# alexandervakhitov/lld-slam

Measured on AMD Instinct MI355X. Metric: local-BA windows/sec (50 KF, 10k pts, 2k lines) at matched chi2; 1/2/4/8 GPU, higher is better.
Workload: dtype f64; 1 GPU; batched LocalBundleAdjustment, 256 LBA-B windows per GPU (50 free + 10 fixed KF, 10k points x 6 stereo obs, 2k lines x 5 KF x 2 images = 80k edges), 5+15 LM iterations, gamma=1; windows resident in HBM, every step restarts from the uploaded state; bit_reproducible=True, windows_per_gpu=256, edges_per_window=80000, parallelism=1 x independent window batches, RCCL gather of result records, resident=True

## Files before the change

lld_slam_amd/csrc/lld_ba_control.h:

```cpp

__device__ __forceinline__ void ba_control_body(const BAArrays& A, const BAWin& W, BAState& S, int lane, int n_windows, int abort_flag,
                                                int wrow , int nw_group ,
                                                int* __restrict__ counters ,
                                                int* __restrict__ host_counters ,
                                                const int* __restrict__ host_abort ) {
  double tempChi = 0.0, scale_l = 0.0;
  int do_clear = 0;
  const bool valid = wrow >= 0;
  if (valid) {
  if (S.phase == PH_RUN) {
    const int nb = W.nt_pt + W.nt_ln;
    for (int i = lane; i < nb; i += 64) { tempChi += xwg_load(&A.chi_part2[W.part_off + i]); scale_l += xwg_load(&A.scale_part[W.part_off + i]); }
    tempChi = lld_wave::sum(tempChi); scale_l = lld_wave::sum(scale_l);
  }
  if (lane == 0 && S.phase == PH_RUN) {
    double scale = S.scale_cam + scale_l;
    if (!S.pcg_ok) tempChi = 1.7976931348623157e308;
    double rho = (S.currentChi - tempChi);
    scale += 1e-3;
    rho /= scale;
    if (rho > 0 && isfinite(tempChi)) {
      double alpha = 1. - (2 * rho - 1) * (2 * rho - 1) * (2 * rho - 1);
      alpha = fmin(alpha, 2. / 3.);
      S.lambda *= fmax(1. / 3., alpha);
      S.ni = 2;
      S.currentChi = tempChi;
      S.cur ^= 1;
    } else {
      S.lambda *= S.ni; S.ni *= 2;
    }
    S.q++;
    const int round = S.round;
    S.lm_trials[round]++;
    const bool stop = abort_flag || (host_abort && __hip_atomic_load(host_abort, __ATOMIC_RELAXED, __HIP_MEMORY_SCOPE_SYSTEM) != 0) ||
                      (W.abort_after > 0 && S.lm_trials[0] + S.lm_trials[1] >= W.abort_after);
    const bool again = (rho < 0 && S.q < W.max_trials && !stop);
    if (!again) {
      bool term = (S.q == W.max_trials || rho == 0);
      if (!term) {
        if ((S.iniChi - S.currentChi) * 1e3 < S.iniChi) S.nBad++; else S.nBad = 0;
        if (S.nBad >= 3) term = true;
      }
      S.it++;
      S.lm_iterations[round]++;
      if (!term && S.it < W.its[round] && !stop) { S.need_lin = 1; S.maxdiag_bits = 0ull; do_clear = 1; }
      else if (round == 0) {
        S.chi2_round1 = S.currentChi; S.chi2_final = S.currentChi;
        if (stop) { S.aborted = 1; S.phase = PH_FINALIZE; }
        else if (W.protocol == 1) S.phase = PH_FINALIZE;
        else S.phase = PH_TRANSITION;
      } else { S.chi2_final = S.currentChi; S.aborted = stop ? 1 : 0; S.phase = PH_FINALIZE; }
    }
  }
  do_clear = __builtin_amdgcn_readfirstlane(do_clear);
  if (do_clear) {
    for (int i = lane; i < W.n_free * 21; i += 64) A.Hpp[(size_t)W.hpp_off * 21 + i] = 0.0;
    for (int i = lane; i < W.n_free * 6; i += 64) A.bp[(size_t)W.hpp_off * 6 + i] = 0.0;
    if (W.big) for (int i = lane; i < W.n_free * 27; i += 64) A.hpp_part[W.hpart_off + i] = 0.0;
  }
  }
  int last = 0;
  if (lane == 0) {
    if (valid) {
      const int ph = S.phase;
      if (ph == PH_RUN) atomicAdd(&counters[0], 1);
      else if (ph == PH_TRANSITION) atomicAdd(&counters[1], 1);
      else if (ph == PH_FINALIZE) atomicAdd(&counters[2], 1);
      if (A.slot_map) { xwg_store_i32(&A.active_pub[wrow], (ph == PH_RUN || ph == PH_TRANSITION) ? 1 : 0); xwg_stores_done(); }
    }
    if (atomicAdd(&counters[3], 1) == n_windows - 1) {
#pragma unroll
      for (int i = 0; i < 3; i++) {
        const int v = atomicExch(&counters[i], 0);
// ... 4 lines not shown
      last = 1;
    }
  }
  last = __builtin_amdgcn_readfirstlane(last);
  if (last && A.slot_map) {
    int cnt = 0;
    for (int base = 0; base < nw_group; base += 64) {
      const int w = base + lane;
      const bool act = w < nw_group && xwg_load_i32(&A.active_pub[w]) != 0;
      const unsigned long long m = __ballot(act);
      if (act) A.slot_map[cnt + __popcll(m & ((1ull << lane) - 1ull))] = w;
      cnt += __popcll(m);
    }
    for (int k = cnt + lane; k < nw_group; k += 64) A.slot_map[k] = -1;
  }
}
__global__ __launch_bounds__(kCtlThreads) void ba_control_kernel(BAArrays A, const BAWin* __restrict__ wins, BAState* __restrict__ st, int abort_flag, int nw_group,
                                                                 int* __restrict__ counters, int* __restrict__ host_counters, const int* __restrict__ host_abort) {
  const int wrow = LLD_ROW_WINDOW(A, st, blockIdx.x);
  const int wi = wrow < 0 ? 0 : wrow;
  ba_control_body(A, wins[wi], st[wi], threadIdx.x, (int)gridDim.x, abort_flag, wrow, nw_group, counters, host_counters, host_abort);
}

__global__ __launch_bounds__(kLmThreads) void ba_backsub_ctl_kernel(BAArrays A, const BAWin* __restrict__ wins, BAState* __restrict__ st, int n_pt_blocks, int abort_flag, int nw_group,
                                                                   int* __restrict__ counters, int* __restrict__ host_counters, const int* __restrict__ host_abort) {
  __shared__ int is_last;
  const int wrow = LLD_ROW_WINDOW(A, st, blockIdx.y);
  const int bx = (int)blockIdx.x;
  if (wrow < 0) {
    if (bx == 0 && threadIdx.x < 64) ba_control_body(A, wins[0], st[0], threadIdx.x, (int)gridDim.y, abort_flag, -1, nw_group, counters, host_counters, host_abort);
    return;
  }
  const BAWin& W = wins[wrow];
  BAState& S = st[wrow];
  const bool running = S.phase == PH_RUN;
  const bool is_pt = bx < n_pt_blocks;
  const bool works = running && (is_pt ? bx < W.nt_pt : bx - n_pt_blocks < W.nt_ln);
  if (works) {
    if (is_pt) ba_backsub_pt_body<false, 1>(A, wins, st, bx); else ba_backsub_ln_body<false, 1>(A, wins, st, bx - n_pt_blocks);
  }
  if (!running) {
    if (bx == 0 && threadIdx.x < 64) ba_control_body(A, W, S, threadIdx.x, (int)gridDim.y, abort_flag, wrow, nw_group, counters, host_counters, host_abort);
    return;
  }
  if (!works) return;
  if (threadIdx.x == 0) is_last = atomicAdd(&S.ticket_bs, 1) == W.nt_pt + W.nt_ln - 1;
  __syncthreads();
  if (is_last && threadIdx.x < 64) {
    if (threadIdx.x == 0) S.ticket_bs = 0;
    ba_control_body(A, W, S, threadIdx.x, (int)gridDim.y, abort_flag, wrow, nw_group, counters, host_counters, host_abort);
  }
}

__global__ __launch_bounds__(kLmThreads) void ba_classify_kernel(BAArrays A, const BAWin* __restrict__ wins, BAState* __restrict__ st) {
  __shared__ double scratch[8];
  const int wrow = LLD_ROW_WINDOW(A, st, blockIdx.y);
  if (wrow < 0) return;
  const BAWin W = wins[wrow];
  BAState& S = st[wrow];
  if (S.phase != PH_TRANSITION) return;
  if ((int)blockIdx.x >= W.nb_pt + W.nb_ln) return;
  const int cur = S.cur;
  const CamK cam = W.cam;
  double n_active = 0.0;
  if ((int)blockIdx.x < W.nb_pt) {
    const int p0 = blockIdx.x * kLmThreads, np = min(kLmThreads, W.n_pt - p0);
    const int eb = A.pt_obs_start[W.pt_off + p0], ee = A.pt_obs_start[W.pt_off + p0 + np];
    for (int e = eb + (int)threadIdx.x; e < ee; e += kLmThreads) {
      uint8_t fl = A.pe_flags[e];
      const Vec3 X = load_pt(A, cur, W.pt_off + A.pe_pt[e]);
      const Pose T = load_cam(A, cur, W.cam_off + pt_cam_of<kPkRuntime>(A, e));
      const bool depth_pos = pose_map(T, X).z > 0.0;
      const bool stereo = pt_obs_stereo<kPkRuntime>(A, e);
      if (A.pe_chi2[e] > (stereo ? 7.815 : 5.991) || !depth_pos) fl |= EF_LEVEL1;
      fl &= (uint8_t)~EF_ROBUST;
      A.pe_flags[e] = fl;
    }
    __syncthreads();
    const int p = p0 + threadIdx.x;
    if (p < W.n_pt) {
      const int g = W.pt_off + p;
      int act = 0;
      for (int e = A.pt_obs_start[g]; e < A.pt_obs_start[g + 1]; e++) act += !(A.pe_flags[e] & EF_LEVEL1);
      A.pt_active[g] = act > 0;
      n_active += act;
    }
  } else {
    const int l0 = (blockIdx.x - W.nb_pt) * kLmThreads, nl = min(kLmThreads, W.n_ln - l0);
    const int eb = 2 * A.ln_obs_start[W.ln_off + l0], ee = 2 * A.ln_obs_start[W.ln_off + l0 + nl];
    for (int e = eb + (int)threadIdx.x; e < ee; e += kLmThreads) {
      uint8_t fl = A.le_flags[e];
      if (!(fl & EF_VALID)) continue;
      const LineQ L = load_ln(A, cur, W.ln_off + ln_line_of<kPkRuntime>(A, e >> 1));
      const Mat3 Rl = line_rotation(L);
      const Vec3 c0 = mat_col(Rl, 0), c1 = mat_col(Rl, 1);
      const double th = (fl & EF_PAIRSTEREO) ? W.th_ln_stereo : W.th_ln_mono;
      const Pose T = load_cam(A, cur, W.cam_off + ln_cam_of<kPkRuntime>(A, e >> 1));
      const LnSeg sg = ln_seg_of<kPkRuntime>(A, e);
      const bool depth_pos = line_depth_positive(cam, (e & 1) ? cam.bx_right : 0.0, T, c0, c1, L.alpha, sg.xs, sg.ys, sg.xe, sg.ye);
      if (A.le_chi2[e] > th * th || !depth_pos) fl |= EF_LEVEL1;
      fl &= (uint8_t)~EF_ROBUST;
      A.le_flags[e] = fl;
    }
    __syncthreads();
    const int l = l0 + threadIdx.x;
    if (l < W.n_ln) {
      const int g = W.ln_off + l;
      const int e0 = 2 * A.ln_obs_start[g], e1 = 2 * A.ln_obs_start[g + 1];
      int cnt = 0, act = 0; bool has_edge = false;
      for (int e = e0; e < e1; e++) {
        const uint8_t fl = A.le_flags[e];
        if (!(fl & EF_VALID)) continue;
        has_edge = true;
        if (!(fl & EF_LEVEL1)) { cnt += 2; act++; }
      }
      const bool removed = has_edge && cnt <= W.ln_filter;
      if (removed) {
        for (int e = e0; e < e1; e++) if (A.le_flags[e] & EF_VALID) A.le_flags[e] |= EF_LEVEL1;
        act = 0;
      }
      A.ln_removed[g] = removed;
      A.ln_active[g] = act > 0;
      n_active += act;
    }
  }
  const double t = block_sum(n_active, scratch);
  __shared__ int is_last;
  if (threadIdx.x == 0) {
    if (t > 0.0) atomicAdd(&S.n_active_edges, (int)(t + 0.5));
    is_last = atomicAdd(&S.ticket_cls, 1) == W.nb_pt + W.nb_ln - 1;
  }
  __syncthreads();
  if (!is_last) return;
  for (int i = threadIdx.x; i < W.n_free * 21; i += kLmThreads) A.Hpp[(size_t)W.hpp_off * 21 + i] = 0.0;
  for (int i = threadIdx.x; i < W.n_free * 6; i += kLmThreads) A.bp[(size_t)W.hpp_off * 6 + i] = 0.0;
  if (W.big) for (int i = threadIdx.x; i < W.n_free * 27; i += kLmThreads) A.hpp_part[W.hpart_off + i] = 0.0;
  __syncthreads();
  if (threadIdx.x == 0) {
    S.ticket_cls = 0;
    S.round = 1; S.it = 0; S.q = 0; S.need_lin = 1; S.maxdiag_bits = 0ull;
    S.phase = __hip_atomic_load(&S.n_active_edges, __ATOMIC_RELAXED, __HIP_MEMORY_SCOPE_AGENT) > 0 ? PH_RUN : PH_FINALIZE;
  }
}

struct BARecordHeader {
  double chi2_round1, chi2_final;
  int lm_iterations[2], lm_trials[2];
  int pcg_iterations, aborted, win_index, n_pt_obs;
};
__device__ __forceinline__ double* rec_cam(unsigned char* r) { return reinterpret_cast<double*>(r + sizeof(BARecordHeader)); }

__global__ __launch_bounds__(kLmThreads) void ba_finalize_kernel(BAArrays A, const BAWin* __restrict__ wins, const BAState* __restrict__ st) {
  const BAWin W = wins[blockIdx.y];
  const BAState& S = st[blockIdx.y];
  if (S.phase != PH_FINALIZE) return;
  if ((int)blockIdx.x >= W.nb_pt + W.nb_ln + 1) return;
  const int cur = S.cur;
  const CamK cam = W.cam;
  const bool global = W.protocol == 1;
  const bool untouched = S.aborted && S.lm_trials[0] == 0;
  unsigned char* rec = A.records + W.rec_off;
  double* o_cam = rec_cam(rec);
  double* o_pt = o_cam + 7 * W.n_cams;
  double* o_x0 = o_pt + 3 * W.n_pt;
  double* o_dir = o_x0 + 3 * W.n_ln;
  unsigned char* o_pe = reinterpret_cast<unsigned char*>(o_dir + 3 * W.n_ln);
  unsigned char* o_le = o_pe + W.n_pe;
  unsigned char* o_rm = o_le + W.n_le;
  if ((int)blockIdx.x == W.nb_pt + W.nb_ln) {
    for (int i = threadIdx.x; i < W.n_cams * 7; i += kLmThreads) o_cam[i] = A.cam_qt[((size_t)cur * A.NC + W.cam_off) * 7 + i];
    if (threadIdx.x == 0) {
      BARecordHeader h;
      h.chi2_round1 = S.chi2_round1; h.chi2_final = S.chi2_final;
      h.lm_iterations[0] = S.lm_iterations[0]; h.lm_iterations[1] = S.lm_iterations[1];
      h.lm_trials[0] = S.lm_trials[0]; h.lm_trials[1] = S.lm_trials[1];
      h.pcg_iterations = S.pcg_iterations; h.aborted = S.aborted; h.win_index = W.win_index; h.n_pt_obs = W.n_pe;
      *reinterpret_cast<BARecordHeader*>(rec) = h;
    }
    return;
  }
  if ((int)blockIdx.x < W.nb_pt) {
    const int p = blockIdx.x * kLmThreads + threadIdx.x;
    if (p < W.n_pt) {
      const Vec3 X = load_pt(A, cur, W.pt_off + p);
      o_pt[3 * p] = X.x; o_pt[3 * p + 1] = X.y; o_pt[3 * p + 2] = X.z;
    }
    for (int e = W.pe_off + p; e < W.pe_off + W.n_pe; e += W.nb_pt * kLmThreads) {
      const Vec3 X = load_pt(A, cur, W.pt_off + A.pe_pt[e]);
      const Pose T = load_cam(A, cur, W.cam_off + pt_cam_of<kPkRuntime>(A, e));
      const bool depth_pos = pose_map(T, X).z > 0.0;
      const bool stereo = pt_obs_stereo<kPkRuntime>(A, e);
      o_pe[e - W.pe_off] = (!untouched && !global && (A.pe_chi2[e] > (stereo ? 7.815 : 5.991) || !depth_pos)) ? 1 : 0;
    }
  } else {
    const int l = (blockIdx.x - W.nb_pt) * kLmThreads + threadIdx.x;
    if (l < W.n_ln) {
      const int g = W.ln_off + l;
      const bool removed = A.ln_removed[g] != 0;
      o_rm[l] = removed;
      if (removed || untouched) {
        for (int k = 0; k < 3; k++) { o_x0[3 * l + k] = A.ln_x0[(size_t)g * 3 + k]; o_dir[3 * l + k] = A.ln_dir[(size_t)g * 3 + k]; }
      } else {
        const LineQ L = load_ln(A, cur, g);
        const Mat3 Rl = line_rotation(L);
        const Vec3 c0 = mat_col(Rl, 0), c1 = mat_col(Rl, 1);
        const Vec3 X1 = L.alpha * c1;
        o_dir[3 * l] = c0.x; o_dir[3 * l + 1] = c0.y; o_dir[3 * l + 2] = c0.z;
        o_x0[3 * l] = X1.x; o_x0[3 * l + 1] = X1.y; o_x0[3 * l + 2] = X1.z;
      }
    }
    for (int e = W.le_off + l; e < W.le_off + W.n_le; e += W.nb_ln * kLmThreads) {
      const int g = W.ln_off + ln_line_of<kPkRuntime>(A, e >> 1);
      const uint8_t fl = A.le_flags[e];
      if (A.ln_removed[g] != 0 || untouched || !(fl & EF_VALID)) { o_le[e - W.le_off] = 0; continue; }
      const LineQ L = load_ln(A, cur, g);
      const Mat3 Rl = line_rotation(L);
      const Vec3 c0 = mat_col(Rl, 0), c1 = mat_col(Rl, 1);
      const Vec3 X1 = L.alpha * c1, X2 = X1 + c0;
      const Pose T = load_cam(A, cur, W.cam_off + ln_cam_of<kPkRuntime>(A, e >> 1));
      const LnSeg sg = ln_seg_of<kPkRuntime>(A, e);
      const double bx = (e & 1) ? cam.bx_right : 0.0;
      const bool depth_pos = line_depth_positive(cam, bx, T, c0, c1, L.alpha, sg.xs, sg.ys, sg.xe, sg.ye);
      double r[2];
      line_residual(cam, bx, pose_map(T, X1), pose_map(T, X2), sg.xs, sg.ys, sg.xe, sg.ye, r, nullptr);
      const double c2 = chi2_of(r, 2, ln_info_of<kPkRuntime>(A, e));
      A.le_chi2[e] = c2;
      const double th = (fl & EF_PAIRSTEREO) ? W.th_ln_stereo : W.th_ln_mono;
      o_le[e - W.le_off] = (!global && (c2 > th * th || !depth_pos)) ? 1 : 0;
    }
  }
}

__global__ void ba_mark_done_kernel(BAState* __restrict__ st, int n_windows) {
  const int w = blockIdx.x * blockDim.x + threadIdx.x;
  if (w < n_windows && st[w].phase == PH_FINALIZE) st[w].phase = PH_DONE;
}
```

lld_slam_amd/csrc/lld_ba_kernels.h:

```cpp
#ifndef LLD_BA_KERNELS_H
#define LLD_BA_KERNELS_H

#include "lld_common.h"
#include "lld_device_math.h"
#include "lld_wave.h"
#include "lld_ba_chol_plan.h"

namespace lldba {

using namespace lld;

constexpr int kLmThreads = 256;
constexpr int kSchurThreads = 64;
constexpr int kSchurWideThreads = 256;
constexpr int kPcgThreads = 1024;
constexpr int kCtlThreads = 64;
constexpr int kLinThreads = 512;
constexpr int kRoundsThroughput[4] = {8, 2, 4, 1};
constexpr int kRoundsLatency[4] = {4, 2, 4, 1};
constexpr int kRoundsThroughputMinWindows = 32;
constexpr int kRoundsThroughputBig[4] = {16, 4, 16, 1};
constexpr int kRoundsBigMinWindows = 192;
constexpr int kAccCopies = 4;
constexpr int kAccCopiesDoc = 4;
constexpr int kMaxFreeCams = 8192;
constexpr int kMaxFreeCamsLds = 590;
constexpr int kMaxFreeCamsOneWg = 170;

enum Phase : int { PH_RUN = 0, PH_TRANSITION = 2, PH_FINALIZE = 3, PH_DONE = 4 };
constexpr uint8_t EF_LEVEL1 = 1, EF_ROBUST = 2, EF_VALID = 4, EF_PAIRSTEREO = 8, EF_STEREO = 16;

struct BAWin {
  CamK cam;
  int n_cams, n_free;
  int cam_off;
  int pt_off, n_pt;
  int ln_off, n_ln;
  int pe_off, n_pe;
  int le_off, n_le;
  int hpp_off;
  int x_off;
  long long S_off;
  int item_off, n_items, n_items_pt;
  int lo_off, n_lo;
  int blk_csr_off, cam_csr_off;
  int n_blk_nz;
  int nb_pt, nb_ln;
  int ptask_off, n_ptasks, nt_pt;
  int ltask_off, n_ltasks, nt_ln;
  int nl_pt, nl_ln;
  int rounds[4];
  long long hpart_off;
  int part_off;
  int its[2];
  int max_trials, ln_filter;
  int abort_after;
  int big;
  int protocol, robust_pts;
  int acc_copies[2];
  int det, lin_waves[2];
  int win_index;
  double th_mono, th_stereo;
  double th_ln_mono, th_ln_stereo;
  long long rec_off;
};

struct BAState {
  int phase, need_lin, round, it, q, cur, nBad, pcg_ok;
  double lambda, ni, currentChi, iniChi, scale_cam;
  unsigned long long maxdiag_bits;
  double chi2_round1, chi2_final;
  int lm_iterations[2], lm_trials[2];
  int pcg_iterations, aborted, n_active_edges, pad;
  int ticket_lin, ticket_bs, ticket_cls, pad2;
};

struct PTask { int l0, nl, e0, ne, ms, pad0, pad1, pad2; };

struct SChunk { int lm_off, n_lm, tab_off, cams_off, k, D, part_off, cpart_off; };

struct BAArrays {
  long long NC, NP, NL;
  double* cam_qt;
  double *ptx, *pty, *ptz;
  double *lqx, *lqy, *lqz, *lqw, *lal;
  const double* cam_qt0;
  const double* pt0;
  const double *ln_x0, *ln_dir;
  const int* pt_obs_start;
  const int* ln_obs_start;
  const int* pe_pt;
  int packed;
  int* slot_map;
  int* active_pub;
  const int* slot_rd;
  const float4* pe_obs;
  const int* pe_cs;
  const float4* lo_seg;
  const int* lo_cs;
  const int* lo_ln;
  const unsigned short* lo_oct;
  const double* ln_info;
  const int* pe_cam;
  const double *pe_u, *pe_v, *pe_ur, *pe_s;
  const int* le_cam; const int* le_ln;
  const double *le_xs, *le_ys, *le_xe, *le_ye, *le_s;
  uint8_t *pe_flags, *le_flags;
  double *pe_chi2, *le_chi2;
  double *pe_ws;
  double *lo_W;
  uint8_t *pt_active, *ln_active, *ln_removed;
  double *pt_V;
  double *ln_V;
  double *hpp_part;
  double *Hpp;
  double *bp;
  double *S, *bschur, *xp;
  double *pcg_vec;
  double *pcg_mi;
  double *pcg_sc;
  long long x_total;
  double *chi_part, *chi_part2, *scale_part;
  const SChunk* sg_chunks;
  const PTask* ptasks; const PTask* ltasks;
  double *sp_part, *sp_cpart;
  const int *blk_start, *blk_src, *cam_start, *cam_src;
// ... 242 lines not shown
```

lld_slam_amd/csrc/lld_ba_lines.h:

```cpp

struct LineGeom { Vec3 c0, c1, X1, X2; double alpha; };
__device__ __forceinline__ LineGeom line_geom(const LineQ& L) {
  const Mat3 Rl = line_rotation_t<true>(L);
  LineGeom G; G.c0 = mat_col(Rl, 0); G.c1 = mat_col(Rl, 1); G.alpha = L.alpha; G.X1 = L.alpha * G.c1; G.X2 = G.X1 + G.c0;
  return G;
}
struct LnObsIn { uint8_t fl[2]; double xs[2], ys[2], xe[2], ye[2], s[2]; };
template <int kPk>
__device__ __forceinline__ void line_obs_load(const BAArrays& A, int o, LnObsIn& I) {
#pragma unroll
  for (int side = 0; side < 2; side++) {
    const int e = 2 * o + side;
    I.fl[side] = A.le_flags[e];
    const LnSeg g = ln_seg_of<kPk>(A, e);
    I.xs[side] = g.xs; I.ys[side] = g.ys; I.xe[side] = g.xe; I.ye[side] = g.ye;
  }
  if (obs_packed<kPk>(A)) { const unsigned oc = A.lo_oct[o]; I.s[0] = A.ln_info[oc & 255u]; I.s[1] = A.ln_info[oc >> 8]; }
  else { I.s[0] = A.le_s[2 * o]; I.s[1] = A.le_s[2 * o + 1]; }
}
__device__ __forceinline__ double line_obs_linearize(const BAArrays& A, const BAWin& W, const Pose& T, int o, int c, const LineGeom& G, const LnObsIn& I,
                                                     double* hb, double* acc_lds) {
  const bool free_cam = c < W.n_free;
  double Wo[24], Jc0[12], r0[2] = {0.0, 0.0}, ws0 = 0.0;
#pragma unroll
  for (int i = 0; i < 24; i++) Wo[i] = 0.0;
#pragma unroll
  for (int i = 0; i < 12; i++) Jc0[i] = 0.0;
  double chi = 0.0;
  const Mat3 Rc = quat_rotation(T.q);
  const Vec3 X1m = pose_map(T, G.X1), X2m = pose_map(T, G.X2);
#pragma unroll
  for (int side = 0; side < 2; side++) {
    const int e = 2 * o + side;
    const uint8_t fl = I.fl[side];
    if (!(fl & EF_VALID) || (fl & EF_LEVEL1)) continue;
    double r[2]; LineAdj adj;
    line_residual_t<true>(W.cam, side == 1 ? W.cam.bx_right : 0.0, X1m, X2m, I.xs[side], I.ys[side], I.xe[side], I.ye[side], r, &adj);
    const double s = I.s[side];
    const double c2 = chi2_of(r, 2, s);
    A.le_chi2[e] = c2;
    double w = 1.0, rho0 = c2;
    if (fl & EF_ROBUST) rho0 = huber_nr(c2, (fl & EF_PAIRSTEREO) ? W.th_ln_stereo : W.th_ln_mono, &w);
    chi += rho0;
    const double ws = w * s;
    double Jc[12], Jl[8];
    line_jac_pose(adj, X1m, X2m, Jc);
    line_jac_line(adj, Rc, G.c0, G.c1, G.alpha, Jl);
    int k = 0;
#pragma unroll
    for (int a = 0; a < 4; a++) {
      hb[10 + a] -= ws * (Jl[a] * r[0] + Jl[4 + a] * r[1]);
#pragma unroll
      for (int d = a; d < 4; d++) hb[k++] += ws * (Jl[a] * Jl[d] + Jl[4 + a] * Jl[4 + d]);
    }
    if (free_cam) {
#pragma unroll
      for (int rr = 0; rr < 6; rr++)
#pragma unroll
        for (int a = 0; a < 4; a++) Wo[rr * 4 + a] += ws * (Jc[rr] * Jl[a] + Jc[6 + rr] * Jl[4 + a]);
      if (side == 0) {
#pragma unroll
        for (int i = 0; i < 12; i++) Jc0[i] = Jc[i];
        r0[0] = r[0]; r0[1] = r[1]; ws0 = ws;
      } else {
        double* ac = acc_lds + c * 27;
        int kk = 0;
#pragma unroll
        for (int rr = 0; rr < 6; rr++) {
          atomicAdd(&ac[21 + rr], -(ws0 * (Jc0[rr] * r0[0] + Jc0[6 + rr] * r0[1]) + ws * (Jc[rr] * r[0] + Jc[6 + rr] * r[1])));
#pragma unroll
          for (int cc = rr; cc < 6; cc++)
            atomicAdd(&ac[kk++], ws0 * (Jc0[rr] * Jc0[cc] + Jc0[6 + rr] * Jc0[6 + cc]) + ws * (Jc[rr] * Jc[cc] + Jc[6 + rr] * Jc[6 + cc]));
        }
        ws0 = 0.0;
      }
    }
  }
  if (free_cam) {
    double* Wb = A.lo_W + (size_t)o * 24;
#pragma unroll
    for (int i = 0; i < 24; i += 2) *reinterpret_cast<double2*>(Wb + i) = make_double2(Wo[i], Wo[i + 1]);
    if (ws0 != 0.0) {
      double* ac = acc_lds + c * 27;
      int kk = 0;
#pragma unroll
      for (int rr = 0; rr < 6; rr++) {
        atomicAdd(&ac[21 + rr], -ws0 * (Jc0[rr] * r0[0] + Jc0[6 + rr] * r0[1]));
#pragma unroll
        for (int cc = rr; cc < 6; cc++) atomicAdd(&ac[kk++], ws0 * (Jc0[rr] * Jc0[cc] + Jc0[6 + rr] * Jc0[6 + cc]));
      }
    }
  }
  return chi;
// ... 55 lines not shown
      const int g = W.ln_off + T.l0;
      if (A.ln_active[g]) {
        const LineGeom G = line_geom(load_ln(A, cur, g));
        for (int sidx = lane; sidx < T.ne; sidx += 64) {
          const int o = T.e0 + sidx, c = ln_cam_of<kPk>(A, o);
          LnObsIn I;
          line_obs_load<kPk>(A, o, I);
          chi += line_obs_linearize(A, W, pose_load(cams + c * 7), o, c, G, I, hb, acc);
        }
        wave_sum_n<14>(hb);
        if (lane == 0) {
          double* V = A.ln_V + (size_t)g * 14;
#pragma unroll
          for (int i = 0; i < 14; i++) V[i] = hb[i];
          maxd = fmax(maxd, fmax(fmax(fabs(hb[0]), fabs(hb[4])), fmax(fabs(hb[7]), fabs(hb[9]))));
        }
      }
    }
  }
  const double chi_t = block_sum(chi, scratch);
  const double max_t = block_max(maxd, scratch);
  if (threadIdx.x == 0) {
    A.chi_part[W.part_off + W.nl_pt + bx] = chi_t;
    atomicMax(&S.maxdiag_bits, (unsigned long long)__double_as_longlong(max_t));
  }
  __syncthreads();
  if (kBig) return;
  double* dst = A.hpp_part + W.hpart_off + (size_t)(W.nl_pt + bx) * nacc;
  for (int i = threadIdx.x; i < nacc; i += nthr) {
    double v = 0.0;
    for (int q = 0; q < copies; q++) v += acc_all[q * nacc + i];
    dst[i] = v;
  }
}
__global__ __launch_bounds__(kLinThreads) void ba_linearize_ln_kernel(BAArrays A, const BAWin* __restrict__ wins, BAState* __restrict__ st) { ba_linearize_ln_body<false, 1>(A, wins, st, (int)blockIdx.x); }
__global__ __launch_bounds__(kLinThreads) void ba_linearize_ln_f64_kernel(BAArrays A, const BAWin* __restrict__ wins, BAState* __restrict__ st) { ba_linearize_ln_body<false, 0>(A, wins, st, (int)blockIdx.x); }
__global__ __launch_bounds__(kLinThreads) void ba_linearize_ln_big_kernel(BAArrays A, const BAWin* __restrict__ wins, BAState* __restrict__ st) { ba_linearize_ln_body<true, kPkRuntime>(A, wins, st, (int)blockIdx.x); }

__device__ __forceinline__ void line_obs_wtx(const BAArrays& A, const BAWin& W, int o, int c, const double* xp, double* t) {
  const double* Wb = A.lo_W + (size_t)o * 24;
#pragma unroll
  for (int k = 0; k < 4; k++) {
    double s = 0.0;
#pragma unroll
    for (int r = 0; r < 6; r++) s += Wb[r * 4 + k] * xp[c * 6 + r];
    t[k] = s;
  }
}
__device__ __forceinline__ double line_obs_trial(const BAArrays& A, const BAWin& W, const Pose& T, int o, const LineGeom& G, const LnObsIn& I) {
  double chi = 0.0;
  const Vec3 X1m = pose_map(T, G.X1), X2m = pose_map(T, G.X2);
#pragma unroll
  for (int side = 0; side < 2; side++) {
    const int e = 2 * o + side;
    const uint8_t fl = I.fl[side];
    if (!(fl & EF_VALID) || (fl & EF_LEVEL1)) continue;
    double r[2];
    line_residual_t<true>(W.cam, side == 1 ? W.cam.bx_right : 0.0, X1m, X2m, I.xs[side], I.ys[side], I.xe[side], I.ye[side], r, nullptr);
    const double c2 = chi2_of(r, 2, I.s[side]);
    A.le_chi2[e] = c2;
    double w, rho0 = c2;
    if (fl & EF_ROBUST) rho0 = huber_nr(c2, (fl & EF_PAIRSTEREO) ? W.th_ln_stereo : W.th_ln_mono, &w);
    chi += rho0;
  }
  return chi;
}
__device__ __forceinline__ double line_backsub(const double* V, double lambda, const double* wtx, const LineQ& L, LineQ& Ln) {
  double t[4], xl[4], sc = 0.0;
#pragma unroll
  for (int i = 0; i < 4; i++) t[i] = V[10 + i] - wtx[i];
  chol_solve<4>(V, lambda, t, xl);
#pragma unroll
  for (int i = 0; i < 4; i++) sc += xl[i] * (lambda * xl[i] + V[10 + i]);
  Ln = line_oplus(L, xl);
  return sc;
}

template <bool kBig, int kPk>
__device__ __forceinline__ void ba_backsub_ln_body(const BAArrays& A, const BAWin* __restrict__ wins, const BAState* __restrict__ st, const int bx) {
  extern __shared__ __attribute__((aligned(16))) double lds[];
  double* scratch = lds;
  const int wrow = LLD_ROW_WINDOW(A, st, blockIdx.y);
  if (wrow < 0) return;
  const BAWin W = wins[wrow];
  const BAState& S = st[wrow];
  if (S.phase != PH_RUN) return;
  if ((int)bx >= W.nt_ln) return;
  const int cur = S.cur, nxt = cur ^ 1;
  const double lambda = S.lambda;
  double* camB_l = lds + 8; double* xps_l = camB_l + W.n_cams * 7;
  const double* camB = kBig ? A.cam_qt + ((size_t)nxt * A.NC + W.cam_off) * 7 : camB_l;
  const double* xp = kBig ? A.xp + W.x_off : xps_l;
  const int task_wave = __builtin_amdgcn_readfirstlane(threadIdx.x >> 6);
  PTask T_next = A.ltasks[W.ltask_off + min((bx * W.rounds[3]) * 4 + task_wave, W.n_ltasks - 1)];
  if (!kBig) {
    for (int i = threadIdx.x; i < W.n_cams * 7; i += kLmThreads) camB_l[i] = A.cam_qt[((size_t)nxt * A.NC + W.cam_off) * 7 + i];
    for (int i = threadIdx.x; i < 6 * W.n_free; i += kLmThreads) xps_l[i] = A.xp[W.x_off + i];
  }
  __syncthreads();
  const int lane = threadIdx.x & 63;
  double chi = 0.0, sc = 0.0;
  for (int rnd = 0; rnd < W.rounds[3]; rnd++) {
    const int ti = (bx * W.rounds[3] + rnd) * 4 + task_wave;
    if (ti >= W.n_ltasks) break;
    const PTask T = T_next;
    T_next = A.ltasks[W.ltask_off + min((bx * W.rounds[3] + rnd + 1) * 4 + task_wave, W.n_ltasks - 1)];
    if (T.nl > 1) {
      const bool has = lane < T.ne;
      const int o = T.e0 + (has ? lane : 0);
      int c, l_raw;
      ln_cam_lm_of<kPk>(A, o, T.l0, c, l_raw);
      LnObsIn I;
      line_obs_load<kPk>(A, o, I);
// ... 126 lines not shown
```

lld_slam_amd/csrc/lld_ba_points.h:

```cpp

__device__ __forceinline__ int dpp_down1(int v) { return __builtin_amdgcn_mov_dpp(v, 0x130, 0xf, 0xf, true); }
__device__ __forceinline__ int dpp_up1(int v) { return __builtin_amdgcn_mov_dpp(v, 0x138, 0xf, 0xf, true); }
template <int OFF>
__device__ __forceinline__ int dpp_down(int v) {
#pragma unroll
  for (int h = 0; h < OFF; h++) v = dpp_down1(v);
  return v;
}
template <int OFF>
__device__ __forceinline__ double dpp_down(double v) {
  return __hiloint2double(dpp_down<OFF>(__double2hiint(v)), dpp_down<OFF>(__double2loint(v)));
}
__device__ __forceinline__ bool seg_step(int seg, int lane, int off) {
  const int so = __shfl_down(seg, off);
  return (lane + off < 64) && so == seg;
}
template <int N, int OFF>
__device__ __forceinline__ void seg_sum_step(double* v, int seg1) {
  const bool ok = dpp_down<OFF>(seg1) == seg1;
  double o[N];
#pragma unroll
  for (int i = 0; i < N; i++) o[i] = dpp_down<OFF>(v[i]);
  if (ok) {
#pragma unroll
    for (int i = 0; i < N; i++) v[i] += o[i];
  }
}
template <int N>
__device__ __forceinline__ void seg_sum(double* v, int seg, int lane, int max_len) {
  if (max_len > 1) seg_sum_step<N, 1>(v, seg + 1);
  if (max_len > 2) seg_sum_step<N, 2>(v, seg + 1);
  if (max_len > 4) seg_sum_step<N, 4>(v, seg + 1);
  for (int off = 8; off < max_len; off <<= 1) {
    const bool ok = seg_step(seg, lane, off);
#pragma unroll
    for (int i = 0; i < N; i++) { const double o = __shfl_down(v[i], off); if (ok) v[i] += o; }
  }
}
template <int N>
__device__ __forceinline__ void wave_sum_n(double* v) {
#pragma unroll
  for (int i = 0; i < N; i++) v[i] = lld_wave::sum(v[i]);
}

struct PtEdgeLin { double r[3], Jp[9], Jc[18], ws, rho0; bool stereo; };

template <int kPk>
__device__ __forceinline__ void point_edge_linearize(const BAArrays& A, const BAWin& W, int cur, int e, uint8_t fl, int c, const Vec3& X, PtEdgeLin& L) {
  const Pose T = load_cam(A, cur, W.cam_off + c);
  const Vec3 Xc = pose_map(T, X);
  const PtObs ob = pt_obs_of<kPk>(A, e);
  L.stereo = !(ob.ur < 0);
  point_residual_iz(W.cam, Xc, rcp_nr(Xc.z), ob.u, ob.v, ob.ur, L.stereo, true, L.r);
  const double s = ob.s;
  const double c2 = chi2_of(L.r, L.stereo ? 3 : 2, s);
  A.pe_chi2[e] = c2;
  double w = 1.0;
  L.rho0 = c2;
  if (fl & EF_ROBUST) L.rho0 = huber_nr(c2, L.stereo ? W.th_stereo : W.th_mono, &w);
  L.ws = w * s;
  A.pe_ws[e] = L.stereo ? -L.ws : L.ws;
  point_jac_point(W.cam, Xc, quat_rotation(T.q), L.stereo, L.Jp);
  point_jac_pose(W.cam, Xc, L.stereo, L.Jc);
}
__device__ __forceinline__ void point_edge_hll(const PtEdgeLin& L, double* hb) {
  int k = 0;
#pragma unroll
  for (int a = 0; a < 3; a++)
#pragma unroll
    for (int d = a; d < 3; d++) hb[k++] = L.ws * (L.Jp[a] * L.Jp[d] + L.Jp[3 + a] * L.Jp[3 + d] + L.Jp[6 + a] * L.Jp[6 + d]);
#pragma unroll
  for (int a = 0; a < 3; a++) hb[6 + a] = -L.ws * (L.Jp[a] * L.r[0] + L.Jp[3 + a] * L.r[1] + L.Jp[6 + a] * L.r[2]);
}
__device__ __forceinline__ void point_edge_hpp(const PtEdgeLin& L, double* ac) {
  int kk = 0;
#pragma unroll
  for (int rr = 0; rr < 6; rr++) {
    atomicAdd(&ac[21 + rr], -L.ws * (L.Jc[rr] * L.r[0] + L.Jc[6 + rr] * L.r[1] + L.Jc[12 + rr] * L.r[2]));
#pragma unroll
    for (int cc = rr; cc < 6; cc++) atomicAdd(&ac[kk++], L.ws * (L.Jc[rr] * L.Jc[cc] + L.Jc[6 + rr] * L.Jc[6 + cc] + L.Jc[12 + rr] * L.Jc[12 + cc]));
  }
}

__device__ __forceinline__ double point_edge_blocks_closed(const BAWin& W, const Pose& T, const Vec3& X, const PtObs& ob, uint8_t fl, double& ws_out,
                                                           double& rho0_out, double* hb, double* hp) {
  const CamK& k = W.cam;
  const Vec3 Xc = pose_map(T, X);
  const bool stereo = !(ob.ur < 0);
  double r[3];
  const double iz = rcp_nr(Xc.z), iz2 = iz * iz;
  point_residual_iz(k, Xc, iz, ob.u, ob.v, ob.ur, stereo, true, r);
  const double c2e = chi2_of(r, stereo ? 3 : 2, ob.s);
  double w = 1.0, rho0 = c2e;
  if (fl & EF_ROBUST) rho0 = huber_nr(c2e, stereo ? W.th_stereo : W.th_mono, &w);
  const double ws = w * ob.s;
  ws_out = ws; rho0_out = rho0;
  const Mat3 R = quat_rotation(T.q);
  const double a = k.fx * iz, b = k.fy * iz;
  const double c0 = -k.fx * Xc.x * iz2, c1 = -k.fy * Xc.y * iz2, c2 = c0 + k.bf * iz2;
  const double m00 = ws * (stereo ? 2.0 * a * a : a * a);
  const double m02 = ws * (stereo ? a * (c0 + c2) : a * c0);
  const double m11 = ws * (b * b), m12 = ws * (b * c1);
  const double m22 = ws * (stereo ? c0 * c0 + c1 * c1 + c2 * c2 : c0 * c0 + c1 * c1);
  const double wr0 = ws * r[0], wr1 = ws * r[1], wr2 = stereo ? ws * r[2] : 0.0;
  const double g0 = a * (wr0 + wr2), g1 = b * wr1, g2 = c0 * wr0 + c1 * wr1 + c2 * wr2;
  double G[3][3];
#pragma unroll
  for (int j = 0; j < 3; j++) {
    G[0][j] = m00 * R.m[0][j] + m02 * R.m[2][j];
// ... 24 lines not shown

template <bool kBig, int kPk>
__device__ __forceinline__ void ba_linearize_pt_body(const BAArrays& A, const BAWin* __restrict__ wins, BAState* __restrict__ st, const int bx) {
  extern __shared__ __attribute__((aligned(16))) double lds[];
  const int wrow = LLD_ROW_WINDOW(A, st, blockIdx.y);
  if (wrow < 0) return;
  const BAWin W = wins[wrow];
  BAState& S = st[wrow];
  if (S.phase != PH_RUN || !S.need_lin) return;
  if ((int)bx >= W.nl_pt) return;
  const int nacc = W.n_free * 27;
  const int cur = S.cur;
  double* acc_all = kBig ? A.hpp_part + W.hpart_off : lds;
  const int copies = W.acc_copies[0];
  double* scratch = kBig ? lds : lds + copies * nacc;
  double* cams_l = scratch + 8;
  const double* cams = kBig ? A.cam_qt + ((size_t)cur * A.NC + W.cam_off) * 7 : cams_l;
  double* acc = acc_all;
  const int nthr = blockDim.x, nwv = W.lin_waves[0];
  const int task_wave = __builtin_amdgcn_readfirstlane(threadIdx.x >> 6);
  PTask T_next = A.ptasks[W.ptask_off + min((bx * W.rounds[0]) * nwv + task_wave, W.n_ptasks - 1)];
  if (!kBig) {
    for (int i = threadIdx.x; i < copies * nacc; i += nthr) acc_all[i] = 0.0;
    acc = acc_all + (W.det ? (int)(threadIdx.x >> 6) : (int)((threadIdx.x >> 3) & (copies - 1))) * nacc;
    for (int i = threadIdx.x; i < W.n_cams * 7; i += nthr) cams_l[i] = A.cam_qt[((size_t)cur * A.NC + W.cam_off) * 7 + i];
  }
  __syncthreads();
  const int lane = threadIdx.x & 63;
  double chi = 0.0, maxd = 0.0;
  for (int rnd = 0; rnd < W.rounds[0]; rnd++) {
    const int ti = (bx * W.rounds[0] + rnd) * nwv + task_wave;
    if (ti >= W.n_ptasks) break;
    const PTask T = T_next;
    T_next = A.ptasks[W.ptask_off + min((bx * W.rounds[0] + rnd + 1) * nwv + task_wave, W.n_ptasks - 1)];
    if (T.nl > 1) {
      const bool has = lane < T.ne;
      const int e = T.e0 + (has ? lane : 0);
      int c, l_raw;
      pt_cam_lm_of<kPk>(A, e, T.l0, c, l_raw);
      const int l = has ? l_raw : -1 - lane;
      const uint8_t fl = A.pe_flags[e];
      const PtObs ob = pt_obs_of<kPk>(A, e);
      const bool lmk = lane < T.nl;
      const int g2 = W.pt_off + T.l0 + (lmk ? lane : 0);
      const Vec3 X2 = load_pt(A, cur, g2);
      const int act2 = lmk ? (int)A.pt_active[g2] : 0;
      const int slot = has ? l - T.l0 : 0;
      Vec3 X; X.x = __shfl(X2.x, slot); X.y = __shfl(X2.y, slot); X.z = __shfl(X2.z, slot);
      const bool lm_act = has && __shfl(act2, slot) != 0;
      const bool head = lm_act && dpp_up1(l + 1) != l + 1;
      double hb[9];
#pragma unroll
      for (int i = 0; i < 9; i++) hb[i] = 0.0;
      if (has && (fl & EF_LEVEL1)) A.pe_ws[e] = 0.0;
      if (lm_act && !(fl & EF_LEVEL1)) {
        double hp[27], ws_e, rho0_e;
        A.pe_chi2[e] = point_edge_blocks_closed(W, pose_load(cams + c * 7), X, ob, fl, ws_e, rho0_e, hb, hp);
        A.pe_ws[e] = (fl & EF_STEREO) ? -ws_e : ws_e;
        chi += rho0_e;
        if (c < W.n_free) {
          double* ac = acc + c * 27;
#pragma unroll
          for (int i = 0; i < 27; i++) if (i != 16) atomicAdd(&ac[i], hp[i]);
        }
      }
      seg_sum<9>(hb, l, lane, T.ms);
      if (head) {
        double* V = A.pt_V + (size_t)(W.pt_off + l) * 9;
#pragma unroll
        for (int i = 0; i < 9; i++) V[i] = hb[i];
        maxd = fmax(maxd, fmax(fabs(hb[0]), fmax(fabs(hb[3]), fabs(hb[5]))));
      }
    } else {
      const int g = W.pt_off + T.l0;
      if (A.pt_active[g]) {
        const Vec3 X = load_pt(A, cur, g);
        double hb[9];
#pragma unroll
        for (int i = 0; i < 9; i++) hb[i] = 0.0;
        for (int sidx = lane; sidx < T.ne; sidx += 64) {
          const int e = T.e0 + sidx;
          const uint8_t fl = A.pe_flags[e];
          if (fl & EF_LEVEL1) { A.pe_ws[e] = 0.0; continue; }
          const int c = pt_cam_of<kPk>(A, e);
          PtEdgeLin L;
          point_edge_linearize<kPk>(A, W, cur, e, fl, c, X, L);
          chi += L.rho0;
          double h1[9];
          point_edge_hll(L, h1);
#pragma unroll
          for (int i = 0; i < 9; i++) hb[i] += h1[i];
          if (c < W.n_free) point_edge_hpp(L, acc + c * 27);
        }
        wave_sum_n<9>(hb);
        if (lane == 0) {
          double* V = A.pt_V + (size_t)g * 9;
#pragma unroll
          for (int i = 0; i < 9; i++) V[i] = hb[i];
          maxd = fmax(maxd, fmax(fabs(hb[0]), fmax(fabs(hb[3]), fabs(hb[5]))));
        }
      }
    }
  }
  const double chi_t = block_sum(chi, scratch);
  const double max_t = block_max(maxd, scratch);
  if (threadIdx.x == 0) {
    A.chi_part[W.part_off + bx] = chi_t;
    atomicMax(&S.maxdiag_bits, (unsigned long long)__double_as_longlong(max_t));
  }
  __syncthreads();
  if (kBig) return;
  double* dst = A.hpp_part + W.hpart_off + (size_t)(bx) * nacc;
  for (int i = threadIdx.x; i < nacc; i += nthr) {
    double v = 0.0;
    for (int q = 0; q < copies; q++) v += acc_all[q * nacc + i];
    dst[i] = v;
  }
}
__global__ __launch_bounds__(kLinThreads, 4) void ba_linearize_pt_kernel(BAArrays A, const BAWin* __restrict__ wins, BAState* __restrict__ st) { ba_linearize_pt_body<false, 1>(A, wins, st, (int)blockIdx.x); }
__global__ __launch_bounds__(kLinThreads, 4) void ba_linearize_pt_f64_kernel(BAArrays A, const BAWin* __restrict__ wins, BAState* __restrict__ st) { ba_linearize_pt_body<false, 0>(A, wins, st, (int)blockIdx.x); }
__global__ __launch_bounds__(kLinThreads, 4) void ba_linearize_pt_big_kernel(BAArrays A, const BAWin* __restrict__ wins, BAState* __restrict__ st) { ba_linearize_pt_body<true, kPkRuntime>(A, wins, st, (int)blockIdx.x); }

__device__ __forceinline__ void point_edge_wtx(const BAArrays& A, const BAWin& W, int cur, int e, uint8_t fl, int c, const Vec3& X, const double* xp, double* t) {
  const double ws = fabs(A.pe_ws[e]);
  const bool stereo = (fl & EF_STEREO) != 0;
  const Pose T = load_cam(A, cur, W.cam_off + c);
  const Vec3 Xc = pose_map(T, X);
  double Jp[9], Jc[18];
  point_jac_point(W.cam, Xc, quat_rotation(T.q), stereo, Jp);
  point_jac_pose(W.cam, Xc, stereo, Jc);
  double uu[3];
#pragma unroll
  for (int i = 0; i < 3; i++) {
    double s = 0.0;
#pragma unroll
    for (int r = 0; r < 6; r++) s += Jc[i * 6 + r] * xp[c * 6 + r];
    uu[i] = ws * s;
  }
#pragma unroll
  for (int k = 0; k < 3; k++) t[k] = Jp[k] * uu[0] + Jp[3 + k] * uu[1] + Jp[6 + k] * uu[2];
}
template <int kPk>
__device__ __forceinline__ double point_edge_trial(const BAArrays& A, const BAWin& W, int nxt, int e, uint8_t fl, int c, const Vec3& Xn) {
  const Pose T = load_cam(A, nxt, W.cam_off + c);
  const Vec3 Xc = pose_map(T, Xn);
  const PtObs ob = pt_obs_of<kPk>(A, e);
  const bool stereo = !(ob.ur < 0);
  double r[3];
  point_residual_iz(W.cam, Xc, rcp_nr(Xc.z), ob.u, ob.v, ob.ur, stereo, true, r);
  const double c2 = chi2_of(r, stereo ? 3 : 2, ob.s);
  A.pe_chi2[e] = c2;
  double w, rho0 = c2;
  if (fl & EF_ROBUST) rho0 = huber_nr(c2, stereo ? W.th_stereo : W.th_mono, &w);
  return rho0;
}
__device__ __forceinline__ double point_backsub(const double* V, double lambda, const double* wtx, const Vec3& X, Vec3& Xn) {
  const double t[3] = {V[6] - wtx[0], V[7] - wtx[1], V[8] - wtx[2]};
  double xl[3], sc = 0.0;
  chol_solve<3>(V, lambda, t, xl);
#pragma unroll
  for (int i = 0; i < 3; i++) sc += xl[i] * (lambda * xl[i] + V[6 + i]);
  Xn = vec3(X.x + xl[0], X.y + xl[1], X.z + xl[2]);
  return sc;
}

template <bool kBig, int kPk>
__device__ __forceinline__ void ba_backsub_pt_body(const BAArrays& A, const BAWin* __restrict__ wins, const BAState* __restrict__ st, const int bx) {
  extern __shared__ __attribute__((aligned(16))) double lds[];
  const int wrow = LLD_ROW_WINDOW(A, st, blockIdx.y);
  if (wrow < 0) return;
  const BAWin W = wins[wrow];
  const BAState& S = st[wrow];
  if (S.phase != PH_RUN) return;
  if ((int)bx >= W.nt_pt) return;
  const int cur = S.cur, nxt = cur ^ 1;
  const double lambda = S.lambda;
  const double* xp = A.xp + W.x_off;
  double* scratch = lds;
  double* camA_l = lds + 8;
  double* camB_l = camA_l + W.n_cams * 7;
  double* xps_l = camB_l + W.n_cams * 7;
  const double* camA = kBig ? A.cam_qt + ((size_t)cur * A.NC + W.cam_off) * 7 : camA_l;
  const double* camB = kBig ? A.cam_qt + ((size_t)nxt * A.NC + W.cam_off) * 7 : camB_l;
  const double* xps = kBig ? xp : xps_l;
  const int task_wave = __builtin_amdgcn_readfirstlane(threadIdx.x >> 6);
  PTask T_next = A.ptasks[W.ptask_off + min((bx * W.rounds[2]) * 4 + task_wave, W.n_ptasks - 1)];
  if (!kBig) {
    for (int i = threadIdx.x; i < W.n_cams * 7; i += kLmThreads) {
      camA_l[i] = A.cam_qt[((size_t)cur * A.NC + W.cam_off) * 7 + i];
      camB_l[i] = A.cam_qt[((size_t)nxt * A.NC + W.cam_off) * 7 + i];
    }
    for (int i = threadIdx.x; i < 6 * W.n_free; i += kLmThreads) xps_l[i] = xp[i];
  }
  __syncthreads();
  const int lane = threadIdx.x & 63;
  double chi = 0.0, sc = 0.0;
  for (int rnd = 0; rnd < W.rounds[2]; rnd++) {
    const int ti = (bx * W.rounds[2] + rnd) * 4 + task_wave;
    if (ti >= W.n_ptasks) break;
    const PTask T = T_next;
    T_next = A.ptasks[W.ptask_off + min((bx * W.rounds[2] + rnd + 1) * 4 + task_wave, W.n_ptasks - 1)];
    if (T.nl > 1) {
      const bool has = lane < T.ne;
      const int e = T.e0 + (has ? lane : 0);
      int c, l_raw;
      pt_cam_lm_of<kPk>(A, e, T.l0, c, l_raw);
      const int l = has ? l_raw : -1 - lane;
      const uint8_t fl = A.pe_flags[e];
      const double ws = fabs(A.pe_ws[e]);
      const PtObs ob = pt_obs_of<kPk>(A, e);
      const bool lmk = lane < T.nl;
      const int g2 = W.pt_off + T.l0 + (lmk ? lane : 0);
      const Vec3 X2 = load_pt(A, cur, g2);
      const int act2 = lmk ? (int)A.pt_active[g2] : 0;
      const int start2 = A.pt_obs_start[g2], end2 = A.pt_obs_start[g2 + 1];
      double V2[9];
#pragma unroll
      for (int i = 0; i < 9; i++) V2[i] = A.pt_V[(size_t)g2 * 9 + i];
      const int slot = has ? l - T.l0 : 0;
      Vec3 X; X.x = __shfl(X2.x, slot); X.y = __shfl(X2.y, slot); X.z = __shfl(X2.z, slot);
      const bool e_act = has && __shfl(act2, slot) != 0 && !(fl & EF_LEVEL1);
      double wtx[3] = {0, 0, 0};
      if (e_act && c < W.n_free) {
        const Pose Tc = pose_load(camA + c * 7);
        const Vec3 Xc = pose_map(Tc, X);
        const bool stereo = (fl & EF_STEREO) != 0;
        const Mat3 R = quat_rotation(Tc.q);
        const double* xc = xps + c * 6;
        const Vec3 v = cross(Xc, vec3(xc[0], xc[1], xc[2])) - vec3(xc[3], xc[4], xc[5]);
        const double iz = rcp_nr(Xc.z), iz2 = iz * iz;
        const double a = W.cam.fx * iz, b = W.cam.fy * iz;
        const double c0 = -W.cam.fx * Xc.x * iz2, c1 = -W.cam.fy * Xc.y * iz2, c2 = c0 + W.cam.bf * iz2;
        const double u0 = ws * (a * v.x + c0 * v.z), u1 = ws * (b * v.y + c1 * v.z), u2 = stereo ? ws * (a * v.x + c2 * v.z) : 0.0;
        const double h0 = a * (u0 + u2), h1 = b * u1, h2 = c0 * u0 + c1 * u1 + c2 * u2;
#pragma unroll
        for (int k = 0; k < 3; k++) wtx[k] = -(R.m[0][k] * h0 + R.m[1][k] * h1 + R.m[2][k] * h2);
      }
      seg_sum<3>(wtx, l, lane, T.ms);
      const int first = (lmk && end2 > start2) ? start2 - T.e0 : 0;
      double wl[3];
#pragma unroll
      for (int i = 0; i < 3; i++) wl[i] = __shfl(wtx[i], first);
      Vec3 Xn2 = X2;
      if (lmk) {
        if (act2 && end2 > start2) sc += point_backsub(V2, lambda, wl, X2, Xn2);
        store_pt(A, nxt, g2, Xn2);
      }
      Vec3 Xn; Xn.x = __shfl(Xn2.x, slot); Xn.y = __shfl(Xn2.y, slot); Xn.z = __shfl(Xn2.z, slot);
      if (e_act) {
        const Vec3 Xc = pose_map(pose_load(camB + c * 7), Xn);
        const bool stereo = !(ob.ur < 0);
        double r[3];
        point_residual_iz(W.cam, Xc, rcp_nr(Xc.z), ob.u, ob.v, ob.ur, stereo, true, r);
        const double c2 = chi2_of(r, stereo ? 3 : 2, ob.s);
        A.pe_chi2[e] = c2;
        double w, rho0 = c2;
        if (fl & EF_ROBUST) rho0 = huber_nr(c2, stereo ? W.th_stereo : W.th_mono, &w);
        chi += rho0;
      }
    } else {
      const int g = W.pt_off + T.l0;
      const Vec3 X = load_pt(A, cur, g);
      if (!A.pt_active[g]) { if (lane == 0) store_pt(A, nxt, g, X); }
      else {
        double wtx[3] = {0, 0, 0};
        for (int sidx = lane; sidx < T.ne; sidx += 64) {
          const int e = T.e0 + sidx;
          const uint8_t fl = A.pe_flags[e];
          const int c = pt_cam_of<kPk>(A, e);
          if ((fl & EF_LEVEL1) || c >= W.n_free) continue;
          double t1[3];
          point_edge_wtx(A, W, cur, e, fl, c, X, xp, t1);
          wtx[0] += t1[0]; wtx[1] += t1[1]; wtx[2] += t1[2];
        }
        wave_sum_n<3>(wtx);
        Vec3 Xn;
        const double s1 = point_backsub(A.pt_V + (size_t)g * 9, lambda, wtx, X, Xn);
        if (lane == 0) { sc += s1; store_pt(A, nxt, g, Xn); }
        for (int sidx = lane; sidx < T.ne; sidx += 64) {
          const int e = T.e0 + sidx;
          const uint8_t fl = A.pe_flags[e];
          if (fl & EF_LEVEL1) continue;
          chi += point_edge_trial<kPk>(A, W, nxt, e, fl, pt_cam_of<kPk>(A, e), Xn);
        }
      }
    }
  }
  const double chi_t = block_sum(chi, scratch);
  const double sc_t = block_sum(sc, scratch);
  if (threadIdx.x == 0) { xwg_store(&A.chi_part2[W.part_off + bx], chi_t); xwg_store(&A.scale_part[W.part_off + bx], sc_t); xwg_stores_done(); }
}
__global__ __launch_bounds__(kLmThreads) void ba_backsub_pt_kernel(BAArrays A, const BAWin* __restrict__ wins, const BAState* __restrict__ st) { ba_backsub_pt_body<false, 1>(A, wins, st, (int)blockIdx.x); }
__global__ __launch_bounds__(kLmThreads) void ba_backsub_pt_f64_kernel(BAArrays A, const BAWin* __restrict__ wins, const BAState* __restrict__ st) { ba_backsub_pt_body<false, 0>(A, wins, st, (int)blockIdx.x); }
__global__ __launch_bounds__(kLmThreads) void ba_backsub_pt_big_kernel(BAArrays A, const BAWin* __restrict__ wins, const BAState* __restrict__ st) { ba_backsub_pt_body<true, kPkRuntime>(A, wins, st, (int)blockIdx.x); }
```

Baseline: 6904 windows/s.

## Recompute per-edge chi2 lazily in classify/finalize instead of storing every iteration

After: 7128 windows/s (median of 6 runs). +3.3%, better.

```diff
diff --git a/lld_slam_amd/csrc/lld_ba_control.h b/lld_slam_amd/csrc/lld_ba_control.h
--- a/lld_slam_amd/csrc/lld_ba_control.h
+++ b/lld_slam_amd/csrc/lld_ba_control.h
@@ -19,6 +19,7 @@
     double rho = (S.currentChi - tempChi);
     scale += 1e-3;
     rho /= scale;
+    S.ev = S.cur ^ 1;
     if (rho > 0 && isfinite(tempChi)) {
       double alpha = 1. - (2 * rho - 1) * (2 * rho - 1) * (2 * rho - 1);
       alpha = fmin(alpha, 2. / 3.);
@@ -129,6 +130,26 @@
   }
 }
 
+__device__ __forceinline__ double point_edge_chi2_at(const BAArrays& A, const BAWin& W, int buf, int e) {
+  const Vec3 Xn = load_pt(A, buf, W.pt_off + A.pe_pt[e]);
+  const Pose T = load_cam(A, buf, W.cam_off + pt_cam_of<kPkRuntime>(A, e));
+  const Vec3 Xc = pose_map(T, Xn);
+  const PtObs ob = pt_obs_of<kPkRuntime>(A, e);
+  const bool stereo = !(ob.ur < 0);
+  double r[3];
+  point_residual_iz(W.cam, Xc, rcp_nr(Xc.z), ob.u, ob.v, ob.ur, stereo, true, r);
+  return chi2_of(r, stereo ? 3 : 2, ob.s);
+}
+__device__ __forceinline__ double line_edge_chi2_at(const BAArrays& A, const BAWin& W, int buf, int e) {
+  const LineGeom G = line_geom(load_ln(A, buf, W.ln_off + ln_line_of<kPkRuntime>(A, e >> 1)));
+  const Pose T = load_cam(A, buf, W.cam_off + ln_cam_of<kPkRuntime>(A, e >> 1));
+  const Vec3 X1m = pose_map(T, G.X1), X2m = pose_map(T, G.X2);
+  const LnSeg sg = ln_seg_of<kPkRuntime>(A, e);
+  double r[2];
+  line_residual_t<true>(W.cam, (e & 1) ? W.cam.bx_right : 0.0, X1m, X2m, sg.xs, sg.ys, sg.xe, sg.ye, r, nullptr);
+  return chi2_of(r, 2, ln_info_of<kPkRuntime>(A, e));
+}
+
 __global__ __launch_bounds__(kLmThreads) void ba_classify_kernel(BAArrays A, const BAWin* __restrict__ wins, BAState* __restrict__ st) {
   __shared__ double scratch[8];
   const int wrow = LLD_ROW_WINDOW(A, st, blockIdx.y);
@@ -137,7 +158,7 @@
   BAState& S = st[wrow];
   if (S.phase != PH_TRANSITION) return;
   if ((int)blockIdx.x >= W.nb_pt + W.nb_ln) return;
-  const int cur = S.cur;
+  const int cur = S.cur, ev = S.ev;
   const CamK cam = W.cam;
   double n_active = 0.0;
   if ((int)blockIdx.x < W.nb_pt) {
@@ -149,9 +170,12 @@
       const Pose T = load_cam(A, cur, W.cam_off + pt_cam_of<kPkRuntime>(A, e));
       const bool depth_pos = pose_map(T, X).z > 0.0;
       const bool stereo = pt_obs_stereo<kPkRuntime>(A, e);
-      if (A.pe_chi2[e] > (stereo ? 7.815 : 5.991) || !depth_pos) fl |= EF_LEVEL1;
+      const double c2 = point_edge_chi2_at(A, W, ev, e);
+      A.pe_chi2[e] = c2;
+      if (c2 > (stereo ? 7.815 : 5.991) || !depth_pos) fl |= EF_LEVEL1;
       fl &= (uint8_t)~EF_ROBUST;
       A.pe_flags[e] = fl;
+      if (fl & EF_LEVEL1) A.pe_ws[e] = 0.0;
     }
     __syncthreads();
     const int p = p0 + threadIdx.x;
@@ -175,7 +199,9 @@
       const Pose T = load_cam(A, cur, W.cam_off + ln_cam_of<kPkRuntime>(A, e >> 1));
       const LnSeg sg = ln_seg_of<kPkRuntime>(A, e);
       const bool depth_pos = line_depth_positive(cam, (e & 1) ? cam.bx_right : 0.0, T, c0, c1, L.alpha, sg.xs, sg.ys, sg.xe, sg.ye);
-      if (A.le_chi2[e] > th * th || !depth_pos) fl |= EF_LEVEL1;
+      const double c2 = line_edge_chi2_at(A, W, ev, e);
+      A.le_chi2[e] = c2;
+      if (c2 > th * th || !depth_pos) fl |= EF_LEVEL1;
       fl &= (uint8_t)~EF_ROBUST;
       A.le_flags[e] = fl;
     }
@@ -232,7 +258,7 @@
   const BAState& S = st[blockIdx.y];
   if (S.phase != PH_FINALIZE) return;
   if ((int)blockIdx.x >= W.nb_pt + W.nb_ln + 1) return;
-  const int cur = S.cur;
+  const int cur = S.cur, ev = S.ev;
   const CamK cam = W.cam;
   const bool global = W.protocol == 1;
   const bool untouched = S.aborted && S.lm_trials[0] == 0;
@@ -267,7 +293,8 @@
       const Pose T = load_cam(A, cur, W.cam_off + pt_cam_of<kPkRuntime>(A, e));
       const bool depth_pos = pose_map(T, X).z > 0.0;
       const bool stereo = pt_obs_stereo<kPkRuntime>(A, e);
-      o_pe[e - W.pe_off] = (!untouched && !global && (A.pe_chi2[e] > (stereo ? 7.815 : 5.991) || !depth_pos)) ? 1 : 0;
+      const double c2 = (untouched || global) ? 0.0 : (A.pe_flags[e] & EF_LEVEL1) ? A.pe_chi2[e] : point_edge_chi2_at(A, W, ev, e);
+      o_pe[e - W.pe_off] = (!untouched && !global && (c2 > (stereo ? 7.815 : 5.991) || !depth_pos)) ? 1 : 0;
     }
   } else {
     const int l = (blockIdx.x - W.nb_pt) * kLmThreads + threadIdx.x;
@@ -301,7 +328,6 @@
       double r[2];
       line_residual(cam, bx, pose_map(T, X1), pose_map(T, X2), sg.xs, sg.ys, sg.xe, sg.ye, r, nullptr);
       const double c2 = chi2_of(r, 2, ln_info_of<kPkRuntime>(A, e));
-      A.le_chi2[e] = c2;
       const double th = (fl & EF_PAIRSTEREO) ? W.th_ln_stereo : W.th_ln_mono;
       o_le[e - W.le_off] = (!global && (c2 > th * th || !depth_pos)) ? 1 : 0;
     }
diff --git a/lld_slam_amd/csrc/lld_ba_kernels.h b/lld_slam_amd/csrc/lld_ba_kernels.h
--- a/lld_slam_amd/csrc/lld_ba_kernels.h
+++ b/lld_slam_amd/csrc/lld_ba_kernels.h
@@ -71,7 +71,8 @@
   unsigned long long maxdiag_bits;
   double chi2_round1, chi2_final;
   int lm_iterations[2], lm_trials[2];
-  int pcg_iterations, aborted, n_active_edges, pad;
+  int pcg_iterations, aborted, n_active_edges;
+  int ev;
   int ticket_lin, ticket_bs, ticket_cls, pad2;
 };
 
diff --git a/lld_slam_amd/csrc/lld_ba_lines.h b/lld_slam_amd/csrc/lld_ba_lines.h
--- a/lld_slam_amd/csrc/lld_ba_lines.h
+++ b/lld_slam_amd/csrc/lld_ba_lines.h
@@ -31,14 +31,12 @@
   const Vec3 X1m = pose_map(T, G.X1), X2m = pose_map(T, G.X2);
 #pragma unroll
   for (int side = 0; side < 2; side++) {
-    const int e = 2 * o + side;
     const uint8_t fl = I.fl[side];
     if (!(fl & EF_VALID) || (fl & EF_LEVEL1)) continue;
     double r[2]; LineAdj adj;
     line_residual_t<true>(W.cam, side == 1 ? W.cam.bx_right : 0.0, X1m, X2m, I.xs[side], I.ys[side], I.xe[side], I.ye[side], r, &adj);
     const double s = I.s[side];
     const double c2 = chi2_of(r, 2, s);
-    A.le_chi2[e] = c2;
     double w = 1.0, rho0 = c2;
     if (fl & EF_ROBUST) rho0 = huber_nr(c2, (fl & EF_PAIRSTEREO) ? W.th_ln_stereo : W.th_ln_mono, &w);
     chi += rho0;
@@ -200,13 +198,11 @@
   const Vec3 X1m = pose_map(T, G.X1), X2m = pose_map(T, G.X2);
 #pragma unroll
   for (int side = 0; side < 2; side++) {
-    const int e = 2 * o + side;
     const uint8_t fl = I.fl[side];
     if (!(fl & EF_VALID) || (fl & EF_LEVEL1)) continue;
     double r[2];
     line_residual_t<true>(W.cam, side == 1 ? W.cam.bx_right : 0.0, X1m, X2m, I.xs[side], I.ys[side], I.xe[side], I.ye[side], r, nullptr);
     const double c2 = chi2_of(r, 2, I.s[side]);
-    A.le_chi2[e] = c2;
     double w, rho0 = c2;
     if (fl & EF_ROBUST) rho0 = huber_nr(c2, (fl & EF_PAIRSTEREO) ? W.th_ln_stereo : W.th_ln_mono, &w);
     chi += rho0;
diff --git a/lld_slam_amd/csrc/lld_ba_points.h b/lld_slam_amd/csrc/lld_ba_points.h
--- a/lld_slam_amd/csrc/lld_ba_points.h
+++ b/lld_slam_amd/csrc/lld_ba_points.h
@@ -54,7 +54,6 @@
   point_residual_iz(W.cam, Xc, rcp_nr(Xc.z), ob.u, ob.v, ob.ur, L.stereo, true, L.r);
   const double s = ob.s;
   const double c2 = chi2_of(L.r, L.stereo ? 3 : 2, s);
-  A.pe_chi2[e] = c2;
   double w = 1.0;
   L.rho0 = c2;
   if (fl & EF_ROBUST) L.rho0 = huber_nr(c2, L.stereo ? W.th_stereo : W.th_mono, &w);
@@ -185,10 +184,9 @@
       double hb[9];
 #pragma unroll
       for (int i = 0; i < 9; i++) hb[i] = 0.0;
-      if (has && (fl & EF_LEVEL1)) A.pe_ws[e] = 0.0;
       if (lm_act && !(fl & EF_LEVEL1)) {
         double hp[27], ws_e, rho0_e;
-        A.pe_chi2[e] = point_edge_blocks_closed(W, pose_load(cams + c * 7), X, ob, fl, ws_e, rho0_e, hb, hp);
+        point_edge_blocks_closed(W, pose_load(cams + c * 7), X, ob, fl, ws_e, rho0_e, hb, hp);
         A.pe_ws[e] = (fl & EF_STEREO) ? -ws_e : ws_e;
         chi += rho0_e;
         if (c < W.n_free) {
@@ -214,7 +212,7 @@
         for (int sidx = lane; sidx < T.ne; sidx += 64) {
           const int e = T.e0 + sidx;
           const uint8_t fl = A.pe_flags[e];
-          if (fl & EF_LEVEL1) { A.pe_ws[e] = 0.0; continue; }
+          if (fl & EF_LEVEL1) continue;
           const int c = pt_cam_of<kPk>(A, e);
           PtEdgeLin L;
           point_edge_linearize<kPk>(A, W, cur, e, fl, c, X, L);
@@ -282,7 +280,6 @@
   double r[3];
   point_residual_iz(W.cam, Xc, rcp_nr(Xc.z), ob.u, ob.v, ob.ur, stereo, true, r);
   const double c2 = chi2_of(r, stereo ? 3 : 2, ob.s);
-  A.pe_chi2[e] = c2;
   double w, rho0 = c2;
   if (fl & EF_ROBUST) rho0 = huber_nr(c2, stereo ? W.th_stereo : W.th_mono, &w);
   return rho0;
@@ -386,7 +383,6 @@
         double r[3];
         point_residual_iz(W.cam, Xc, rcp_nr(Xc.z), ob.u, ob.v, ob.ur, stereo, true, r);
         const double c2 = chi2_of(r, stereo ? 3 : 2, ob.s);
-        A.pe_chi2[e] = c2;
         double w, rho0 = c2;
         if (fl & EF_ROBUST) rho0 = huber_nr(c2, stereo ? W.th_stereo : W.th_mono, &w);
         chi += rho0;
```
